# Chyaboiii/antidote_ccrdt

Measured on AMD Instinct MI355X. Metric: CRDT ops/sec (topk_rmv, 1M keys, 8-DC vclocks), higher is better.
Workload: dtype int64

## Files before the change

antidote_ccrdt_amd/csrc/engine.cpp:

```cpp
#include <algorithm>
#include <chrono>
#include <cstdio>
#include <cstdlib>
#include <cstring>
#include <string>
#include <thread>
#include <tuple>
#include <vector>

#include "common.hpp"
#include "engine.hpp"
#include "trmv_kernels.hpp"

namespace ccrdt {

static thread_local std::string g_last_error;
void set_error(const std::string& msg) { g_last_error = msg; }

static constexpr int TRMV_N_TIERS = CCRDT_TRMV_N_TIERS;
static constexpr int TRMV_TIER_LAST = CCRDT_TRMV_TIER_HBM;
static constexpr uint32_t TRMV_HBM_WAVES = 128;
static constexpr uint32_t TRMV_LATER_GRID = 4096;

template <class F>
// ... 234 lines not shown
  }
  if (e->type != CCRDT_TOPK_RMV) {
    set_error("engine is not topk_rmv");
    return CCRDT_ENOSYS;
  }
  if (hipSetDevice(e->device) != hipSuccess) {
    set_error("hipSetDevice failed");
    return CCRDT_EDEVICE;
  }
  return CCRDT_OK;
}

namespace {

int trmv_err_code(uint32_t err) {
  std::string m = "trmv_apply: invalid op in batch:";
  if (err & TRMV_ERR_KIND) m += " kind>3";
  if (err & TRMV_ERR_DC) m += " dc>=n_dc";
  if (err & TRMV_ERR_TS) m += " add ts<1";
  if (err & TRMV_ERR_ROW) m += " rmv row out of range";
  if (err & TRMV_ERR_VC) m += " negative VcRmv entry";
  set_error(m);
  return (err & (TRMV_ERR_TS | TRMV_ERR_VC)) && !(err & (TRMV_ERR_KIND | TRMV_ERR_DC | TRMV_ERR_ROW)) ? CCRDT_ERANGE
                                                                                                  : CCRDT_EINVAL;
}

int env_int(const char* v, int dflt, int lo, int hi) { return std::clamp(v ? atoi(v) : dflt, lo, hi); }
bool env_on(const char* v) { return !(v && v[0] == '0'); }
bool env_is1(const char* v) { return v && v[0] == '1'; }
uint64_t env_u64(const char* v, uint64_t dflt) { return v ? strtoull(v, nullptr, 10) : dflt; }
struct TrmvKnobs {
  int pool_slack = env_int(getenv("CCRDT_TRMV_POOL_SLACK"), 2, 2, 8);
  int first_tier = env_int(getenv("CCRDT_TRMV_FIRST_TIER"), -1, INT32_MIN, INT32_MAX);
  bool overlap = env_on(getenv("CCRDT_TRMV_OVERLAP"));
  bool inplace = env_on(getenv("CCRDT_TRMV_INPLACE"));
  uint64_t overlap_keys = env_u64(getenv("CCRDT_TRMV_OVERLAP_KEYS"), 1ull << 18);
  uint32_t overlap_waves = (uint32_t)env_int(getenv("CCRDT_TRMV_OVERLAP_WAVES"), 32, 1, 4096);
  static const TrmvKnobs& get() {
    static const TrmvKnobs k;
    return k;
  }
};
struct TrmvHooks {
  static bool fail_finish() { return env_is1(getenv("CCRDT_TRMV_FAIL_FINISH")); }
  static bool overlap_stall() { return env_is1(getenv("CCRDT_TRMV_OVERLAP_STALL")); }
  static const char* arena_room() { return getenv("CCRDT_TRMV_ARENA_ROOM"); }
};

struct TrmvStatus {
  static constexpr int TRMV_STATUS_WORDS = 2 + 2 * TRMV_N_TIERS;
  static constexpr uint64_t ALLOC = TRMV_STATUS_WORDS * 4 + 16;
  uint32_t* dev;
  uint32_t* host;
  hipStream_t stream;
  uint32_t* count(int t) const { return dev + 2 + 2 * t; }
  uint32_t* verr() const { return count(CCRDT_TRMV_TIER_RESIDENT) + 1; }
  unsigned long long* vscratch() const { return reinterpret_cast<unsigned long long*>(dev + TRMV_STATUS_WORDS); }
  hipError_t clear() const { return hipMemsetAsync(dev, 0, TRMV_STATUS_WORDS * 4, stream); }
  hipError_t clear_tier(int t) const { return hipMemsetAsync(count(t), 0, 8, stream); }
  hipError_t read_back(bool sync = true) const {
    const hipError_t e = hipMemcpyAsync(host, dev, TRMV_STATUS_WORDS * 4, hipMemcpyDeviceToHost, stream);
    return e != hipSuccess || !sync ? e : hipStreamSynchronize(stream);
  }
  uint32_t handed(int t) const { return host[2 + 2 * t]; }
  uint32_t errors(int t) const { return host[3 + 2 * t]; }
};

struct TrmvRun {
  Engine& E;
  TrmvStatus st;
  TrmvApplyArgs a;
  uint64_t n_ops;
  uint64_t tot[3] = {};
  int chain[4] = {}, n_chain = 0, n_head = 0;
  int prev = -1;
  int next_evt = 0;
};
// ... 227 lines not shown
  a0.n_first = ov + O_NFIRST;
  a0.first_thresh = thresh;
  CCRDT_TRY(trmv_launch_wave(a0, nk, E.stream));
  CCRDT_TRY(trmv_mark(r));
  CCRDT_HIP(hipStreamWaitEvent(E.stream2, E.evt[e0], 0));
  trmv_point(E, r.st, a3, CCRDT_TRMV_TIER_RESIDENT, CCRDT_TRMV_TIER_WAVE);
  a3.prod_waves = trmv_wave_waves(nk);
  a3.claim = ov + O_CLAIM;
  const bool force_stall = TrmvHooks::overlap_stall();
  a3.spin_limit = force_stall ? 0u : (1u << 19);
  CCRDT_TRY(trmv_launch_resident_consume(a3, TrmvKnobs::get().overlap_waves, E.stream2));
  CCRDT_HIP(hipEventRecord(E.ev_ovl, E.stream2));
  CCRDT_HIP(hipStreamWaitEvent(E.stream, E.ev_ovl, 0));
  CCRDT_TRY(trmv_mark(r));
  CCRDT_HIP(r.st.read_back());
  if ((r.st.errors(CCRDT_TRMV_TIER_RESIDENT) & TRMV_ERR_STALL) || force_stall) {
    CCRDT_HIP(r.st.clear_tier(CCRDT_TRMV_TIER_RESIDENT));
    a3.pub = nullptr;
    a3.done = nullptr;
    CCRDT_TRY(trmv_launch_resident(a3, std::min<uint64_t>(nk, TRMV_LATER_GRID), E.stream));
    --r.next_evt;
    CCRDT_TRY(trmv_mark(r));
    CCRDT_HIP(r.st.read_back());
    E.trmv_overflow_keys[CCRDT_TRMV_SLOT_STALL_FALLBACK] = 1;
  }
  CCRDT_TRY(trmv_book(E, r.st, r.chain, 2, e0));
  r.prev = CCRDT_TRMV_TIER_RESIDENT;
  return CCRDT_OK;
}

int trmv_run_chain(TrmvRun& r) {
  const Engine& E = r.E;
  const TrmvKnobs& knobs = TrmvKnobs::get();
  const bool overlap = knobs.overlap && E.fresh && E.n_keys && (uint64_t)E.n_keys <= knobs.overlap_keys &&
                       r.n_head == 2 && r.chain[0] == CCRDT_TRMV_TIER_WAVE && r.chain[1] == CCRDT_TRMV_TIER_RESIDENT;
  if (overlap) CCRDT_TRY(trmv_head_overlapped(r));
  else CCRDT_TRY(trmv_segment(r, r.chain, r.n_head));
  if (r.n_head < r.n_chain && E.n_keys && r.st.handed(r.chain[r.n_head - 1]) != 0)
    CCRDT_TRY(trmv_segment(r, r.chain + r.n_head, r.n_chain - r.n_head));
  return CCRDT_OK;
}

int trmv_tier4_and_keep(TrmvRun& r, int& n_over) {
  Engine& E = r.E;
  const uint32_t n_big = E.n_keys ? r.st.handed(CCRDT_TRMV_TIER_S1024) : 0u;
  if (n_big) {
    CCRDT_TRY(E.hbm_scratch.ensure((uint64_t)TRMV_HBM_WAVES * trmv_steady_hbm_bytes(E.k <= 128)));
    const int tier_hbm = CCRDT_TRMV_TIER_HBM;
    r.prev = CCRDT_TRMV_TIER_S1024;
    CCRDT_TRY(trmv_segment(r, &tier_hbm, 1, n_big));
  }
  n_over = (int)E.trmv_overflow_keys[CCRDT_TRMV_TIER_HBM];
  if (n_over) {
    r.a.key_list = E.tier_ovf[TRMV_TIER_LAST].as<uint32_t>();
    r.a.n_list = 0;
    r.a.n_list_dev = r.st.count(TRMV_TIER_LAST);
    CCRDT_TRY(trmv_launch_keep(r.a, std::min<uint32_t>((uint32_t)n_over, TRMV_LATER_GRID), E.stream));
  }
  return CCRDT_OK;
}

int trmv_open_arena(TrmvRun& r) {
  Engine& E = r.E;
  const uint64_t* tot = r.tot;
  trmv_side_caps(E, 1 - E.cur, E.arena_cap);
  if (const char* v = TrmvHooks::arena_room())
    for (int x = 0; x < 3; ++x) E.arena_cap[x] = std::min<uint64_t>(E.arena_cap[x], tot[x] + strtoull(v, nullptr, 10));
// ... 917 lines not shown
```

antidote_ccrdt_amd/csrc/trmv_wave.hip:

```cpp
#include "common.hpp"
#include "trmv_kernels.hpp"

#ifdef TRMV_PROF
__device__ unsigned long long g_trmv_prof[16];
#define PROF_STAMP(v)                                                        \
  do {                                                                       \
    __builtin_amdgcn_sched_barrier(0);                                       \
    asm volatile("s_memtime %0\n\ts_waitcnt lgkmcnt(0)" : "=s"(v)::"memory"); \
    __builtin_amdgcn_sched_barrier(0);                                       \
  } while (0)
#define PROF_MARK(i)                                                         \
  do {                                                                       \
    unsigned long long _t;                                                   \
    PROF_STAMP(_t);                                                          \
    if (lane_id() == 0 && (key & 63u) == 3) atomicAdd(&g_trmv_prof[i], _t - prof_t);             \
    prof_t = _t;                                                             \
  } while (0)
#else
#define PROF_STAMP(v) (void)0
#define PROF_MARK(i) (void)0
#endif

namespace ccrdt {

// ... 18 lines not shown
  unsigned long long htab[W_HCAP + 2];
  int64_t esc[W_ECAP + 2];
  int64_t ets[W_ECAP + 2];
  int64_t rows[W_RCAP][TRMV_DPAD];
  unsigned long long vc[TRMV_DPAD + 2];
  uint32_t pcnt2[W_PCAP / 2 + 4];
  uint32_t rsrc[W_RCAP];
  uint16_t ekd[W_ECAP + 8];
  uint8_t hp[W_HCAP];
  uint8_t sorted[W_ECAP + 8];
  uint8_t slab[W_ECAP];
  uint8_t fin[NS_ * (W_ECAP + 8)];
  uint32_t pa[W_PCAP + 8];
  uint32_t pb[W_PCAP + 8];
  uint8_t pmoff[NS_ * (W_PCAP + 8)];
  uint8_t peb[NS_ * (W_PCAP + 8)];
  uint8_t cpl[W_PCAP + 8];
  uint8_t rl[W_RCAP + 8];
  uint32_t nex;
  __device__ __forceinline__ uint8_t& fa(uint32_t p, int b) { return reinterpret_cast<uint8_t*>(pa)[4 * p + b]; }
  __device__ __forceinline__ uint8_t& fb(uint32_t p, int b) { return reinterpret_cast<uint8_t*>(pb)[4 * p + b]; }
};
#define PSTART(p) L.fa((p), 0)
#define PLR(p) L.fa((p), 1)
#define PFLAG(p) L.fa((p), 2)
#define PCNTF(p) L.fa((p), 3)
#define POBS(p) L.fb((p), 0)
#define PROW(p) L.fb((p), 1)
#define PGB(p) L.fb((p), 2)
#define PSLOT(p) L.fb((p), 3)

#define KA trmv_kargs()

__device__ __forceinline__ uint32_t whash(int64_t id) {
  const uint64_t x = (uint64_t)id * 0x9E3779B97F4A7C15ull;
  return (uint32_t)(x >> 56);
}

template <class W>
__device__ __forceinline__ uint32_t pcnt_of(const W& L, uint32_t p) {
  return (L.pcnt2[p >> 1] >> (16 * (p & 1))) & 0xFFFFu;
}

template <class W>
__device__ __forceinline__ void wave_emit(const TrmvApplyArgs& a, W& L, uint64_t op0,
                                          uint64_t op, uint8_t kind, int64_t id, int64_t sc,
                                          uint32_t dc, int64_t ts, uint32_t row) {
  const uint32_t pos = atomicAdd(&L.nex, 1u);
  TrmvExtraRec r;
  r.op = (uint32_t)op;
  r.kind = kind;
  r.dc = (uint8_t)dc;
  r.pad = 0;
  r.id = id;
  r.score = sc;
  r.ts = ts;
  KA->ex[op0 + pos] = r;
  if (kind == CCRDT_TRMV_RMV)
    for (int d = 0; d < KA->n_dc; ++d) KA->ex_vc[(op0 + pos) * KA->n_dc + d] = L.rows[row][d];
}

struct KeyIn {
  uint64_t op0;
  uint32_t nops;
  KeyMeta nmeta;
  int64_t id[2], sc[2], ts[2];
  uint32_t kind[2], dc[2];
  int64_t rv[W_RCAP / 8];
};

struct ChunkHdr {
  uint32_t key;
  uint64_t lo, hi;
  uint32_t meta[W_MD];
  uint64_t skip;
};

__device__ __forceinline__ uint32_t wave_list_key(uint32_t i, uint32_t n_first) {
  if (KA->first_list) return i < n_first ? KA->first_list[i] : i - n_first;
  return KA->key_list ? KA->key_list[i] : i;
}

__device__ __forceinline__ void wave_load_chunk(const TrmvApplyArgs& a, uint32_t c0, uint32_t n,
                                                uint32_t n_first, ChunkHdr& h) {
  const int lane = lane_id();
  const uint32_t j = (uint32_t)lane < n ? (uint32_t)lane : 0u;
  h.key = wave_list_key(c0 + j, n_first);
  h.lo = KA->key_ptr[h.key];
  h.hi = KA->key_ptr[h.key + 1];
  h.skip = KA->first_list ? ballot((uint32_t)lane < n && c0 + j >= n_first && h.hi - h.lo > KA->first_thresh) : 0ull;
#pragma unroll
  for (int i = 0; i < W_MD; ++i) {
    const uint32_t m = 8 * i + (lane >> 3);
    const uint32_t jm = m < n ? m : 0u;
    const uint32_t km = shfl32(h.key, (int)jm);
    if (KA->fresh) {
      const uint32_t d = lane & 7;
      h.meta[i] = d < 3 ? (uint32_t)trmv_fresh_off(KA->slack != 0, (int)d, km, KA->key_ptr[km])
                        : (d == 7 ? NONE32 : 0u);
    } else {
      h.meta[i] = reinterpret_cast<const uint32_t*>(a.new_s.meta + km)[lane & 7];
    }
  }
}

__device__ __forceinline__ void wave_load_key(const TrmvApplyArgs& a, const ChunkHdr& h, uint32_t j,
                                              KeyIn& in) {
  const int lane = lane_id();
  in.op0 = (uint64_t)rl64((int64_t)h.lo, (int)j);
  in.nops = (uint32_t)((uint64_t)rl64((int64_t)h.hi, (int)j) - in.op0);
  uint32_t* m = reinterpret_cast<uint32_t*>(&in.nmeta);
#pragma unroll
  for (int d = 0; d < 8; ++d) {
    uint32_t v = 0;
#pragma unroll
    for (int i = 0; i < W_MD; ++i)
      if ((j >> 3) == (uint32_t)i) v = rl32(h.meta[i], (int)(8 * (j & 7) + d));
    m[d] = v;
  }
  const int64_t* idp = KA->id + in.op0;
  const int64_t* scp = KA->score + in.op0;
  const int64_t* tsp = KA->ts + in.op0;
  const uint8_t* kp = KA->kind + in.op0;
  const uint8_t* dp = KA->dc + in.op0;
#pragma unroll
  for (int s = 0; s < 2; ++s) {
    const uint32_t l = s * 64 + lane;
    const bool v = l < in.nops;
    in.id[s] = v ? LD_IN(idp + l) : 0;
    in.sc[s] = v ? LD_IN(scp + l) : 0;
    in.ts[s] = v ? LD_IN(tsp + l) : 0;
    in.kind[s] = v ? (uint32_t)LD_IN(kp + l) : 0u;
    in.dc[s] = v ? (uint32_t)LD_IN(dp + l) : 0u;
  }
}

template <class W>
__device__ __forceinline__ void wave_load_rows(const TrmvApplyArgs& a, W& L, KeyIn& in) {
  const int lane = lane_id();
#pragma unroll
  for (int s = 0; s < W_RCAP / 8; ++s) in.rv[s] = 0;
  bool r[2];
#pragma unroll
  for (int s = 0; s < 2; ++s)
    r[s] = (uint32_t)(s * 64 + lane) < in.nops && (in.kind[s] == 2 || in.kind[s] == 3);
  const uint64_t b0 = ballot(r[0]), b1 = ballot(r[1]);
  const uint32_t n0 = (uint32_t)__builtin_popcountll(b0);
  const uint32_t n = n0 + (uint32_t)__builtin_popcountll(b1);
  if (n == 0 || KA->n_rmv_rows <= 0) return;
#pragma unroll
  for (int s = 0; s < 2; ++s) {
    const uint32_t k = s ? n0 + mbcnt(b1) : mbcnt(b0);
    if (r[s] && k < (uint32_t)W_RCAP)
      L.rsrc[k] = (in.ts[s] >= 0 && in.ts[s] < KA->n_rmv_rows) ? (uint32_t)in.ts[s] : 0u;
  }
  wave_lds_sync();
  const uint32_t d = (lane & 7) < KA->n_dc ? (lane & 7) : 0u;
#pragma unroll
  for (int s = 0; s < W_RCAP / 8; ++s) {
    const uint32_t k = s * 8 + (lane >> 3);
    const uint32_t row = k < n ? L.rsrc[k] : 0u;
    in.rv[s] = KA->rmv_vc[(uint64_t)row * KA->n_dc + d];
  }
  wave_lds_sync();
}

enum : int { W_DONE = 0, W_NEXT_TIER = 1, W_REJECT = 2 };

template <bool FRESH>
__device__ __forceinline__ int trmv_wave_key(const TrmvApplyArgs& a, uint32_t key, const KeyIn& in,
                                              WaveLds<FRESH>& L, bool has_next, const ChunkHdr& hdr,
                                              uint32_t nj, KeyIn& nxt) {
  int lane = lane_id();
  asm volatile("" : "+v"(lane));
  const int D = KA->n_dc;
#ifdef TRMV_PROF
  unsigned long long prof_t;
  PROF_STAMP(prof_t);
#endif
  const uint64_t op0 = in.op0;
  const uint32_t nops = in.nops;
  KeyMeta nmeta = in.nmeta;
  nmeta.p_off = __builtin_amdgcn_readfirstlane(nmeta.p_off);
  nmeta.m_off = __builtin_amdgcn_readfirstlane(nmeta.m_off);
  nmeta.r_off = __builtin_amdgcn_readfirstlane(nmeta.r_off);
  KeyMeta om;
  if (FRESH) {
    om.p_off = om.m_off = om.r_off = 0;
    om.np = om.nm = om.nr = om.nobs = 0;
    om.minq = NONE32;
  } else {
    om = a.old_s.meta[key];
  }
  const uint32_t pmax = KA->k < (uint32_t)W_PCAP ? KA->k : (uint32_t)W_PCAP;
  if (nops > (uint32_t)W_ECAP || om.np > pmax || om.nm + nops > (uint32_t)W_ECAP ||
      om.nr > (uint32_t)W_RCAP)
    return W_NEXT_TIER;

  int64_t xsc[2] = {in.sc[0], in.sc[1]};
  const int64_t xts[2] = {in.ts[0], in.ts[1]};
  const uint32_t xkind[2] = {in.kind[0], in.kind[1]};
  const uint32_t xdc[2] = {in.dc[0], in.dc[1]};
  const bool xv[2] = {(uint32_t)lane < nops, (uint32_t)(64 + lane) < nops};
  int64_t pid[2] = {0, 0};
  uint32_t pinfo[2] = {NONE32, NONE32}, pslab[2] = {0u, 0u};
  if (!FRESH) {
#pragma unroll
    for (int s = 0; s < 2; ++s) {
      const uint32_t p = s * 64 + lane;
      if (p < om.np) {
        pid[s] = (a.old_s.pl_id + om.p_off)[p];
        pinfo[s] = (a.old_s.pl_info + om.p_off)[p];
        pslab[s] = (a.old_s.pl_slab + om.p_off)[p];
      }
    }
  }
#pragma unroll
  for (int i = 0; i < W_HCAP / 64; ++i) L.htab[i * 64 + lane] = W_EMPTY;
  if (lane == 0) {
    L.htab[HSINK] = W_EMPTY;
    L.nex = 0u;
  }
  reinterpret_cast<uint32_t*>(L.hp)[lane] = 0xFFFFFFFFu;
  L.pcnt2[lane] = 0u;
  L.pa[lane] = 0u;
  L.pa[64 + lane] = 0u;
  L.pb[lane] = 0xFFFFFFFFu;
  L.pb[64 + lane] = 0xFFFFFFFFu;
  if (lane < 8) {
    L.pa[128 + lane] = 0u;
    L.pb[128 + lane] = 0xFFFFFFFFu;
  }
  if (lane < TRMV_DPAD)
    L.vc[lane] = (!FRESH && lane < D) ? (unsigned long long)a.old_s.vc[(uint64_t)key * D + lane] : 0ull;
  if (!FRESH) {
    for (uint32_t r0 = 0; r0 < om.nr; r0 += 8) {
      const uint32_t r = r0 + (lane >> 3), d = lane & 7;
      if (r < om.nr)
        L.rows[r][d] = (int)d < D ? (a.old_s.r_vc + (uint64_t)om.r_off * D)[r * D + d] : 0;
    }
  }

  PROF_MARK(0);
  uint32_t err = 0;
  bool xr[2], xa[2];
#pragma unroll
  for (int s = 0; s < 2; ++s) {
    xa[s] = xv[s] && xkind[s] < 2;
    xr[s] = xv[s] && (xkind[s] == 2 || xkind[s] == 3);
    err |= (xv[s] && xkind[s] > 3) ? TRMV_ERR_KIND : 0u;
    err |= (xa[s] && (int)xdc[s] >= D) ? TRMV_ERR_DC : 0u;
    err |= (xa[s] && xts[s] < 1) ? TRMV_ERR_TS : 0u;
    err |= (xr[s] && (xts[s] < 0 || xts[s] >= KA->n_rmv_rows)) ? TRMV_ERR_ROW : 0u;
  }
  if (ballot(err != 0)) {
    if (err) atomicOr(&KA->status[1], err);
    return W_REJECT;
  }
  const uint64_t rb0 = ballot(xr[0]), rb1 = ballot(xr[1]);
  const uint32_t nr0 = (uint32_t)__builtin_popcountll(rb0);
  const uint32_t nrmv = nr0 + (uint32_t)__builtin_popcountll(rb1);
  if (om.nr + nrmv > (uint32_t)W_RCAP) return W_NEXT_TIER;
  {
    const uint32_t r0 = mbcnt(rb0), r1 = nr0 + mbcnt(rb1);
    xsc[0] = xr[0] ? (int64_t)(om.nr + r0) : xsc[0];
    xsc[1] = xr[1] ? (int64_t)(om.nr + r1) : xsc[1];
  }
  wave_lds_sync();
  constexpr int NS = FRESH ? 2 : 4;
  uint32_t hs[4];
  bool pend[4];
  const int64_t hid[4] = {in.id[0], in.id[1], pid[0], pid[1]};
  pend[0] = xv[0];
  pend[1] = xv[1];
  pend[2] = !FRESH && (uint32_t)lane < om.np;
  pend[3] = !FRESH && (uint32_t)(64 + lane) < om.np;
  bool bad = false;
#pragma unroll
  for (int j = 0; j < NS; ++j) {
    hs[j] = whash(hid[j]);
    bad |= pend[j] && (unsigned long long)hid[j] == W_EMPTY;
  }
  if (ballot(bad)) return W_NEXT_TIER;

  PROF_MARK(1);
  for (;;) {
    bool any = false;
#pragma unroll
    for (int j = 0; j < NS; ++j) any |= pend[j];
    if (!ballot(any)) break;
    unsigned long long prev[4];
#pragma unroll
    for (int j = 0; j < NS; ++j) {
      prev[j] = W_EMPTY;
      if (pend[j]) prev[j] = atomicCAS(&L.htab[hs[j]], W_EMPTY, (unsigned long long)hid[j]);
    }
#pragma unroll
    for (int j = 0; j < NS; ++j) {
      const bool done = prev[j] == W_EMPTY || prev[j] == (unsigned long long)hid[j];
      hs[j] = (pend[j] && !done) ? ((hs[j] + 1) & (W_HCAP - 1)) : hs[j];
      pend[j] = pend[j] && !done;
    }
  }
  PROF_MARK(8);
  {
#pragma unroll
    for (int s = 0; s < W_RCAP / 8; ++s) {
      const uint32_t r = s * 8 + (lane >> 3), d = lane & 7;
      const int64_t v = (int)d < D ? in.rv[s] : 0;
      err |= (r < nrmv && v < 0) ? TRMV_ERR_VC : 0u;
      if (r < nrmv) L.rows[om.nr + r][d] = v;
    }
    if (ballot(err != 0)) {
      if (err) atomicOr(&KA->status[1], err);
      return W_REJECT;
    }
  }
  PROF_MARK(9);
  if (!FRESH) {
#pragma unroll
    for (int s = 0; s < 2; ++s) {
      const uint32_t p = s * 64 + lane;
      if (p < om.np) {
        L.hp[hs[2 + s]] = (uint8_t)p;
        PSLOT(p) = (uint8_t)hs[2 + s];
        bad |= ((pslab[s] >> 16) != 0) != ((pinfo[s] & 0xFFFFu) != NONE16);
      }
    }
    if (ballot(bad)) return W_NEXT_TIER;
  }
  wave_lds_sync();
  uint32_t np;
  {
    const unsigned long long* h4 = &L.htab[lane * 4];
    const unsigned long long t0 = h4[0], t1 = h4[1], t2 = h4[2], t3 = h4[3];
    const uint32_t hp4 = reinterpret_cast<const uint32_t*>(L.hp)[lane];
    const uint32_t n0 = (t0 != W_EMPTY && (hp4 & 0xFFu) == NONE8) ? 1u : 0u;
    const uint32_t n1 = (t1 != W_EMPTY && ((hp4 >> 8) & 0xFFu) == NONE8) ? 1u : 0u;
    const uint32_t n2 = (t2 != W_EMPTY && ((hp4 >> 16) & 0xFFu) == NONE8) ? 1u : 0u;
    const uint32_t n3 = (t3 != W_EMPTY && (hp4 >> 24) == NONE8) ? 1u : 0u;
    const uint32_t c = n0 + n1 + n2 + n3;
    const uint64_t b0 = ballot(c & 1), b1 = ballot(c & 2), b2 = ballot(c & 4);
    const uint32_t base = om.np + mbcnt(b0) + 2 * mbcnt(b1) + 4 * mbcnt(b2);
    np = om.np + (uint32_t)__builtin_popcountll(b0) + 2 * (uint32_t)__builtin_popcountll(b1) +
         4 * (uint32_t)__builtin_popcountll(b2);
    if (np > pmax) return W_NEXT_TIER;
    const uint32_t i0 = base, i1 = i0 + n0, i2 = i1 + n1, i3 = i2 + n2;
    const uint32_t nhp = (n0 ? i0 : (hp4 & 0xFFu)) | ((n1 ? i1 : ((hp4 >> 8) & 0xFFu)) << 8) |
                         ((n2 ? i2 : ((hp4 >> 16) & 0xFFu)) << 16) |
                         ((n3 ? i3 : (hp4 >> 24)) << 24);
    reinterpret_cast<uint32_t*>(L.hp)[lane] = nhp;
    if (n0) PSLOT(i0) = (uint8_t)(lane * 4 + 0);
    if (n1) PSLOT(i1) = (uint8_t)(lane * 4 + 1);
    if (n2) PSLOT(i2) = (uint8_t)(lane * 4 + 2);
    if (n3) PSLOT(i3) = (uint8_t)(lane * 4 + 3);
  }
  wave_lds_sync();
  if (FRESH && has_next) wave_load_key(a, hdr, nj, nxt);

  PROF_MARK(2);
  uint32_t xrank[2], xp[2];
  {
    uint32_t hpv[2], cr[2];
#pragma unroll
    for (int s = 0; s < 2; ++s) hpv[s] = L.hp[hs[s]];
#pragma unroll
    for (int s = 0; s < 2; ++s) {
      const uint32_t p = xv[s] ? hpv[s] : PSINK;
      xp[s] = p;
      if (xa[s]) atomicMax(&L.vc[xdc[s]], (unsigned long long)xts[s]);
      if (!FRESH && xr[s]) PFLAG(p) = 1;
      cr[s] = atomicAdd(&L.pcnt2[(xv[s] ? p : (uint32_t)lane) >> 1], xv[s] ? 1u << (16 * (p & 1)) : 0u);
    }
#pragma unroll
    for (int s = 0; s < 2; ++s) xrank[s] = xv[s] ? (cr[s] >> (16 * (xp[s] & 1))) & 0xFFFFu : 0u;
  }
  wave_lds_sync();
  {
    uint32_t tot0, tot1;
    const uint32_t c0 = (uint32_t)lane < np ? pcnt_of(L, lane) : 0u;
    const uint32_t c1 = (uint32_t)(64 + lane) < np ? pcnt_of(L, 64 + lane) : 0u;
    const uint32_t st0 = wave_excl_scan_dpp(c0, tot0);
    const uint32_t st1 = wave_excl_scan_dpp(c1, tot1);
    PSTART(lane) = (uint8_t)st0;
    PSTART(64 + lane) = (uint8_t)(tot0 + st1);
  }
  wave_lds_sync();
  uint32_t xq[2], xst[2], xc[2];
#pragma unroll
  for (int s = 0; s < 2; ++s) {
    xst[s] = PSTART(xp[s]);
// ... 40 lines not shown
      wave_lds_sync();
#pragma unroll
      for (int s = 0; s < 2; ++s)
        if (xv[s])
          for (uint32_t x = 0; x < xc[s]; ++x)
            if (L.sorted[xst[s] + x] == (uint32_t)(s * 64 + lane)) xq[s] = xst[s] + x;
    }
  }
  if (!FRESH) {
    uint32_t ebase = nops;
#pragma unroll
    for (int s = 0; s < 2; ++s) {
      const uint32_t p = s * 64 + lane;
      const uint32_t oc = p < om.np ? (pslab[s] >> 16) : 0u;
      uint32_t tot;
      const uint32_t eb = ebase + wave_excl_scan_dpp(oc, tot);
      ebase += tot;
      if (p < om.np) {
        L.peb[p] = (uint8_t)eb;
        PFLAG(p) = 1;
      }
      for (uint32_t j = 0; j < oc; ++j) {
        const uint32_t go = (pslab[s] & 0xFFFFu) + j;
        const uint32_t e = eb + j;
        L.esc[e] = (a.old_s.m_score + om.m_off)[go];
        L.ets[e] = (a.old_s.m_ts + om.m_off)[go];
        L.ekd[e] = (uint16_t)(((uint32_t)(a.old_s.m_dc + om.m_off)[go] << 2) | (p << 8));
      }
    }
  }
  wave_lds_sync();

  PROF_MARK(3);
  if (!FRESH && has_next) wave_load_key(a, hdr, nj, nxt);
  if (!FRESH) {
    bool simple[2], beaten[2] = {false, false}, gbeaten[2] = {false, false}, risk[2] = {false, false};
    uint32_t me[2], cl[2];
#pragma unroll
    for (int s = 0; s < 2; ++s) {
      simple[s] = xa[s] && !PFLAG(xp[s]);
      me[s] = xq[s] - xst[s];
      cl[s] = simple[s] ? xc[s] : 0u;
    }
    const uint32_t maxc = wave_max_u32_dpp(cl[0] > cl[1] ? cl[0] : cl[1]);
    for (uint32_t x = 0; x < maxc; ++x) {
#pragma unroll
      for (int s = 0; s < 2; ++s) {
        const bool valid = x < cl[s] && x != me[s];
        const uint32_t pos = x < cl[s] ? xst[s] + x : (uint32_t)ESINK;
        const int64_t sx = L.esc[pos], tx = L.ets[pos];
        const uint32_t dx = (L.ekd[pos] >> 2) & 7u;
        const int64_t sm = xsc[s], tm = xts[s];
        const bool before = x < me[s];
        risk[s] |= valid && before && tx >= tm;
        beaten[s] |= valid && (sx > sm || (sx == sm && (before ? tx >= tm : tx > tm)));
        gbeaten[s] |= valid && (sx > sm || (sx == sm && (dx > xdc[s] || (dx == xdc[s] && tx > tm))));
      }
    }
#pragma unroll
    for (int s = 0; s < 2; ++s) {
      if (risk[s]) PFLAG(xp[s]) = 1;
      if (simple[s] && !beaten[s]) POBS(xp[s]) = (uint8_t)xq[s];
      if (simple[s] && !gbeaten[s]) PGB(xp[s]) = (uint8_t)xq[s];
    }
    wave_lds_sync();
  } else {
    uint8_t* const cq = L.slab;
// ... 71 lines not shown
      if (act) mrg[k] = (uint8_t)(yr && !first);
      any_merge |= ballot(yr && !first) != 0;
    }
    wave_lds_sync();
    if (any_merge) {
#pragma unroll 1
      for (uint32_t b = 0; b < mn; b += 64) {
        const uint32_t k = b + lane;
        const uint32_t q = k < mn && mrg[k] ? (uint32_t)cq[k] : ESINK;
        const uint32_t p = q != ESINK ? (uint32_t)(L.ekd[q] >> 8) : PSINK;
        if (q != ESINK && !PFLAG(p)) {
          unsigned long long* dst = reinterpret_cast<unsigned long long*>(L.rows[PROW(p)]);
          const int64_t* src = L.rows[(uint32_t)L.esc[q]];
          for (int d = 0; d < D; ++d) atomicMax(dst + d, (unsigned long long)src[d]);
        }
      }
    }
    wave_lds_sync();
  }

  PROF_MARK(6);
  uint32_t ncx;
  {
    const bool c0 = (uint32_t)lane < np && PFLAG(lane);
    const bool c1 = (uint32_t)(64 + lane) < np && PFLAG(64 + lane);
    const uint64_t m0 = ballot(c0), m1 = ballot(c1);
    const uint32_t n0 = (uint32_t)__builtin_popcountll(m0);
    ncx = n0 + (uint32_t)__builtin_popcountll(m1);
    if (c0) L.cpl[mbcnt(m0)] = (uint8_t)lane;
    if (c1) L.cpl[n0 + mbcnt(m1)] = (uint8_t)(64 + lane);
  }
  wave_lds_sync();
  __builtin_amdgcn_s_waitcnt(0x0F70);
  if (FRESH && has_next) wave_load_rows(a, L, nxt);
  PROF_MARK(7);
  uint32_t best_q = NONE32;
  int64_t best_sc = INT64_MAX, best_id = INT64_MAX;
  auto min_cand = [&](bool has, int64_t sc, int64_t id, uint32_t p) {
    const bool better = has && (best_q == NONE32 || sc < best_sc || (sc == best_sc && id < best_id));
    best_q = better ? p : best_q;
    best_sc = better ? sc : best_sc;
    best_id = better ? id : best_id;
  };
  if (FRESH) {
#pragma unroll
    for (int s = 0; s < 2; ++s) {
      const uint32_t q = s * 64 + lane;
      const uint32_t qq = q < nops ? q : (uint32_t)ESINK;
      const int64_t sc = L.esc[qq], ts = L.ets[qq];
      const uint32_t kd = L.ekd[qq];
      if (q < nops) {
        ST_OUT((KA->new_s.m_score + nmeta.m_off) + (q), sc);
        ST_OUT((KA->new_s.m_ts + nmeta.m_off) + (q), ts);
        ST_OUT((KA->new_s.m_dc + nmeta.m_off) + (q), (uint8_t)((kd >> 2) & 7u));
      }
    }
  }
  uint32_t mbase = 0;
#pragma unroll 1
  for (uint32_t b = 0; b < ncx; b += 64) {
    const uint32_t k = b + lane;
    const bool act = k < ncx;
    const uint32_t p = act ? L.cpl[k] : 0u;
    uint32_t ocnt = 0, pinfo_p = NONE32, eb = 0;
    if (!FRESH && act && p < om.np) {
      pinfo_p = (a.old_s.pl_info + om.p_off)[p];
      ocnt = (a.old_s.pl_slab + om.p_off)[p] >> 16;
      eb = L.peb[p];
    }
    const uint32_t c = act ? pcnt_of(L, p) : 0u;
    const uint32_t st = act ? PSTART(p) : 0u;
    uint32_t tot;
    const uint32_t moff = mbase + wave_excl_scan_dpp(c + ocnt, tot);
    mbase += tot;
    uint32_t cnt = ocnt;
    int64_t maxts = 0;
    for (uint32_t j = 0; j < cnt; ++j) {
      L.slab[moff + j] = (uint8_t)(eb + j);
      const int64_t t = L.ets[eb + j];
      maxts = t > maxts ? t : maxts;
    }
    uint32_t o = NONE8, prow = NONE8;
    int64_t osc = 0, ots = 0;
    if (!FRESH && act && p < om.np) {
      const uint32_t oi = pinfo_p & 0xFFFFu, ri = pinfo_p >> 16;
      if (oi != NONE16) {
        o = eb + oi;
// ... 45 lines not shown
        bool alive = false;
        int64_t bsc = 0, bts = 0;
        for (uint32_t j = 0; j < cnt; ++j) {
          const uint32_t e2 = L.slab[moff + j];
          const int64_t t2 = L.ets[e2];
          const uint32_t d2 = (L.ekd[e2] >> 2) & 7u;
          if (t2 > L.rows[vs][d2]) {
            L.slab[moff + w++] = (uint8_t)e2;
            alive |= e2 == o;
            const int64_t s2 = L.esc[e2];
            if (be == NONE8 || s2 > bsc || (s2 == bsc && (d2 > bdc || (d2 == bdc && t2 > bts)))) {
              be = e2;
              bsc = s2;
              bdc = d2;
              bts = t2;
            }
          }
        }
        cnt = w;
        if (o != NONE8 && !alive) {
          if (cnt == 0) {
            o = NONE8;
          } else {
            o = be;
            osc = bsc;
            ots = bts;
            wave_emit(a, L, op0, op0 + L.sorted[e], CCRDT_TRMV_ADD, id, bsc, bdc, bts, prow);
          }
        }
      }
    }
    if (FRESH) {
      uint32_t opos = NONE16, gj = 0;
      for (uint32_t j = 0; j < cnt; ++j) {
        const uint32_t e2 = L.slab[moff + j];
        const int64_t s2 = L.esc[e2], t2 = L.ets[e2];
        const uint32_t d2 = (L.ekd[e2] >> 2) & 7u;
        ST_OUT((KA->new_s.m_score + nmeta.m_off) + (st + j), s2);
        ST_OUT((KA->new_s.m_ts + nmeta.m_off) + (st + j), t2);
        ST_OUT((KA->new_s.m_dc + nmeta.m_off) + (st + j), (uint8_t)d2);
        opos = e2 == o ? j : opos;
        const uint32_t eb = L.slab[moff + gj];
        const int64_t bs = L.esc[eb], bt = L.ets[eb];
        const uint32_t bd = (L.ekd[eb] >> 2) & 7u;
        if (s2 > bs || (s2 == bs && (d2 > bd || (d2 == bd && t2 > bt)))) gj = j;
      }
      if (act) {
        POBS(p) = (uint8_t)(o == NONE8 ? NONE8 : st + opos);
        PGB(p) = (uint8_t)(st + gj);
        PCNTF(p) = (uint8_t)cnt;
        PROW(p) = (uint8_t)prow;
      }
      min_cand(act && o != NONE8, osc, id, p);
    } else if (act) {
      POBS(p) = (uint8_t)o;
      PCNTF(p) = (uint8_t)cnt;
      L.pmoff[p] = (uint8_t)moff;
      PROW(p) = (uint8_t)prow;
    }
  }
  wave_lds_sync();
  if (!FRESH && has_next) wave_load_rows(a, L, nxt);

  PROF_MARK(4);
  uint32_t fbase = 0, rbase = 0, nobs = 0;
  uint32_t po[2] = {NONE8, NONE8};
  if (FRESH) {
    uint32_t csum = 0;
#pragma unroll
    for (int s = 0; s < 2; ++s) {
      const uint32_t p = s * 64 + lane;
      const bool act = p < np;
      const uint32_t pp = act ? p : (uint32_t)PSINK;
      const uint32_t wa = L.pa[pp], wb = L.pb[pp];
      const uint32_t st = wa & 0xFFu, c = pcnt_of(L, pp), lrp = (wa >> 8) & 0xFFu;
      const bool replayed = ((wa >> 16) & 0xFFu) != 0;
      const uint32_t off = (replayed || lrp == 0) ? st : lrp;
      const uint32_t cnt = act ? (replayed ? (wa >> 24) : st + c - off) : 0u;
      const uint32_t o = act ? (wb & 0xFFu) : NONE8;
      const uint32_t prow = act ? ((wb >> 8) & 0xFFu) : NONE8;
      const uint64_t rm = ballot(prow != NONE8);
      const uint32_t rix = rbase + mbcnt(rm);
      rbase += (uint32_t)__builtin_popcountll(rm);
      if (prow != NONE8) L.rl[rix] = (uint8_t)prow;
      const int64_t id = (int64_t)L.htab[wb >> 24];
      const uint32_t gb = (replayed || cnt > 1) ? ((wb >> 16) & 0xFFu) - off : 0u;
      if (act) {
        ST_OUT((KA->new_s.pl_id + nmeta.p_off) + (p), id);
        ST_OUT((KA->new_s.pl_slab + nmeta.p_off) + (p), off | (cnt << 16));
        if (cnt > 1) ST_OUT((KA->new_s.pl_gb + nmeta.p_off) + (p), (uint16_t)gb);
        ST_OUT(KA->new_s.pl_info + nmeta.p_off + p, (o == NONE8 ? NONE16 : o - off) |
                                             ((prow != NONE8 ? rix : NONE16) << 16));
      }
      csum += cnt;
      nobs += (uint32_t)__builtin_popcountll(ballot(o != NONE8));
      min_cand(!replayed && o != NONE8, L.esc[o != NONE8 ? o : (uint32_t)ESINK], id, p);
    }
    (void)wave_excl_scan_dpp(csum, fbase);
    wave_lds_sync();
  } else {
  {
    uint32_t cnt[2], st[2], moff[2], goff[2], prow[2], opos[2], gbj[2], gbd[2];
    int64_t gbs[2], gbt[2];
    bool act[2], cx[2];
#pragma unroll
    for (int s = 0; s < 2; ++s) {
      const uint32_t p = s * 64 + lane;
      act[s] = p < np;
      const uint32_t pp = act[s] ? p : PSINK;
      cx[s] = act[s] && PFLAG(pp);
      const uint32_t c = pcnt_of(L, pp);
      st[s] = PSTART(pp);
      po[s] = act[s] ? POBS(pp) : NONE8;
      cnt[s] = act[s] ? (cx[s] ? (uint32_t)PCNTF(pp) : c) : 0u;
      prow[s] = cx[s] ? PROW(pp) : NONE8;
      moff[s] = cx[s] ? L.pmoff[pp] : 0u;
      uint32_t ftot;
      goff[s] = fbase + wave_excl_scan_dpp(cnt[s], ftot);
      fbase += ftot;
      opos[s] = (act[s] && !cx[s]) ? po[s] - st[s] : NONE16;
      gbj[s] = (act[s] && !cx[s]) ? (uint32_t)PGB(pp) - st[s] : 0u;
      gbd[s] = 0u;
      gbs[s] = gbt[s] = 0;
    }
    const uint32_t maxcnt = wave_max_u32_dpp(cnt[0] > cnt[1] ? cnt[0] : cnt[1]);
// ... 21 lines not shown
      const uint32_t p = s * 64 + lane;
      const uint64_t rm = ballot(prow[s] != NONE8);
      const uint32_t rix = rbase + mbcnt(rm);
      rbase += (uint32_t)__builtin_popcountll(rm);
      if (prow[s] != NONE8) L.rl[rix] = (uint8_t)prow[s];
      const int64_t id = (int64_t)L.htab[PSLOT(act[s] ? p : PSINK)];
      if (act[s]) {
        (KA->new_s.pl_id + nmeta.p_off)[p] = id;
        (KA->new_s.pl_info + nmeta.p_off)[p] = (po[s] == NONE8 ? NONE16 : opos[s]) |
                                             ((prow[s] != NONE8 ? rix : NONE16) << 16);
        (KA->new_s.pl_slab + nmeta.p_off)[p] = goff[s] | (cnt[s] << 16);
        (KA->new_s.pl_gb + nmeta.p_off)[p] = (uint16_t)(cnt[s] ? gbj[s] : 0u);
      }
      nobs += (uint32_t)__builtin_popcountll(ballot(act[s] && po[s] != NONE8));
    }
  }
  wave_lds_sync();

#pragma unroll
  for (int s = 0; s < 2; ++s) {
    const uint32_t q = s * 64 + lane;
    const uint32_t e0 = L.fin[q < fbase ? q : (uint32_t)ESINK];
    const uint32_t e = e0 < (uint32_t)W_ECAP ? e0 : (uint32_t)ESINK;
    const int64_t sc = L.esc[e], ts = L.ets[e];
    const uint8_t dc = (uint8_t)((L.ekd[e] >> 2) & 7u);
    if (q < fbase) {
      (KA->new_s.m_score + nmeta.m_off)[q] = sc;
      (KA->new_s.m_ts + nmeta.m_off)[q] = ts;
      (KA->new_s.m_dc + nmeta.m_off)[q] = dc;
    }
  }
  }
  PROF_MARK(10);
  for (uint32_t r0 = 0; r0 < rbase; r0 += 8) {
    const uint32_t r = r0 + (lane >> 3), d = lane & 7;
    const int64_t v = L.rows[L.rl[r < rbase ? r : 0u]][d];
    if (r < rbase && (int)d < D) (KA->new_s.r_vc + (uint64_t)nmeta.r_off * D)[r * D + d] = v;
  }
  if (lane < D) KA->new_s.vc[(uint64_t)key * D + lane] = (int64_t)L.vc[lane];
  PROF_MARK(11);
  {
    if (!FRESH) {
#pragma unroll
      for (int s = 0; s < 2; ++s) {
        const uint32_t p = s * 64 + lane;
        const uint32_t o = po[s];
        const int64_t sc = L.esc[o != NONE8 ? o : (uint32_t)ESINK];
        const int64_t id = (int64_t)L.htab[PSLOT(o != NONE8 ? p : (uint32_t)PSINK)];
        min_cand(o != NONE8, sc, id, p);
      }
    }
    const bool has = best_q != NONE32;
    const bool narrow = best_sc == (int64_t)(int32_t)best_sc && best_id == (int64_t)(int32_t)best_id;
    if (!ballot(has)) {
      best_q = NONE32;
    } else if (!ballot(has && !narrow)) {
      const uint32_t us = has ? (uint32_t)(int32_t)best_sc ^ 0x80000000u : 0xFFFFFFFFu;
      const uint32_t ms = wave_min_u32_dpp(us);
      const bool at = has && us == ms;
      const uint32_t ui = at ? (uint32_t)(int32_t)best_id ^ 0x80000000u : 0xFFFFFFFFu;
      const uint32_t mi = wave_min_u32_dpp(ui);
      best_q = rl32(best_q, (int)__builtin_ctzll(ballot(at && ui == mi)));
    } else {
      const int64_t ms = wave_min_i64_dpp(has ? best_sc : INT64_MAX);
      const int64_t mi = wave_min_i64_dpp(has && best_sc == ms ? best_id : INT64_MAX);
      const uint64_t hit = ballot(has && best_sc == ms && best_id == mi);
      best_q = rl32(best_q, (int)__builtin_ctzll(hit));
    }
  }
  if (lane == 0) {
    KeyMeta out = nmeta;
    out.np = np;
    out.nm = fbase;
    out.nr = rbase;
    out.nobs = nobs;
    out.minq = best_q;
    KA->new_s.meta[key] = out;
    KA->ex_cnt[key] = L.nex;
    if (FRESH && KA->slack) {
      KeyCap c;
      c.p_cap = trmv_fresh_cap(true, 0, nops);
      c.m_cap = trmv_fresh_cap(true, 1, nops);
      c.r_cap = trmv_fresh_cap(true, 2, nops);
      c.m_top = (uint16_t)nops;
      c.flags = TRMV_CAP_VALID;
      KA->new_s.cap[key] = c;
    }
  }
  PROF_MARK(5);
  return W_DONE;
}
}

template <bool FRESH, int OCC>
__global__ __launch_bounds__(64 * W_WAVES, OCC) void trmv_wave_kernel(TrmvApplyArgs a) {
  __shared__ WaveLds<FRESH> lds[W_WAVES];
  const uint32_t wv = __builtin_amdgcn_readfirstlane(threadIdx.x >> 6);
  WaveLds<FRESH>& L = lds[wv];
  const uint32_t n_first = a.first_list ? *a.n_first : 0u;
  const uint32_t n = (a.n_list_dev ? *a.n_list_dev : a.n_list) + n_first;
  for (uint32_t c0 = (blockIdx.x * W_WAVES + wv) * W_KPW; c0 < n; c0 += gridDim.x * W_WAVES * W_KPW) {
    const uint32_t cn = c0 + W_KPW < n ? W_KPW : n - c0;
    ChunkHdr hdr;
    wave_load_chunk(a, c0, cn, n_first, hdr);
    KeyIn cur, nxt;
    wave_load_key(a, hdr, 0, cur);
    __builtin_amdgcn_s_waitcnt(0x0F70);
    wave_load_rows(a, L, cur);
    for (uint32_t j = 0; j < cn; ++j) {
      const uint32_t key = rl32(hdr.key, (int)j);
      const bool has_next = j + 1 < cn;
      const int r = (hdr.skip >> j) & 1u ? W_REJECT + 1
                                         : trmv_wave_key<FRESH>(a, key, cur, L, has_next, hdr, j + 1, nxt);
      if (r != W_DONE) {
        if (r == W_NEXT_TIER && lane_id() == 0) {
          const uint32_t pos = atomicAdd(&KA->status[0], 1u);
          KA->ovf_list[pos] = key;
          if (KA->pub && pos < KA->n_pub) {
            const uint32_t old = atomicExch(&KA->pub[pos], key + 1u);
// ... 52 lines not shown
```

Baseline: 47.81 billion.

## Hoist kernel-arg loads, use 32-bit offset addressing, and reorder next-key prefetch

Result: faster. 49.79 billion, median of 6 (+4.1%).

```diff
diff --git a/antidote_ccrdt_amd/csrc/engine.cpp b/antidote_ccrdt_amd/csrc/engine.cpp
--- a/antidote_ccrdt_amd/csrc/engine.cpp
+++ b/antidote_ccrdt_amd/csrc/engine.cpp
@@ -290,7 +290,6 @@
 struct TrmvKnobs {
   int pool_slack = env_int(getenv("CCRDT_TRMV_POOL_SLACK"), 2, 2, 8);
   int first_tier = env_int(getenv("CCRDT_TRMV_FIRST_TIER"), -1, INT32_MIN, INT32_MAX);
-  bool overlap = env_on(getenv("CCRDT_TRMV_OVERLAP"));
   bool inplace = env_on(getenv("CCRDT_TRMV_INPLACE"));
   uint64_t overlap_keys = env_u64(getenv("CCRDT_TRMV_OVERLAP_KEYS"), 1ull << 18);
   uint32_t overlap_waves = (uint32_t)env_int(getenv("CCRDT_TRMV_OVERLAP_WAVES"), 32, 1, 4096);
@@ -301,6 +300,7 @@
 };
 struct TrmvHooks {
   static bool fail_finish() { return env_is1(getenv("CCRDT_TRMV_FAIL_FINISH")); }
+  static bool overlap() { return env_on(getenv("CCRDT_TRMV_OVERLAP")); }
   static bool overlap_stall() { return env_is1(getenv("CCRDT_TRMV_OVERLAP_STALL")); }
   static const char* arena_room() { return getenv("CCRDT_TRMV_ARENA_ROOM"); }
 };
@@ -594,7 +594,7 @@
 int trmv_run_chain(TrmvRun& r) {
   const Engine& E = r.E;
   const TrmvKnobs& knobs = TrmvKnobs::get();
-  const bool overlap = knobs.overlap && E.fresh && E.n_keys && (uint64_t)E.n_keys <= knobs.overlap_keys &&
+  const bool overlap = TrmvHooks::overlap() && E.fresh && E.n_keys && (uint64_t)E.n_keys <= knobs.overlap_keys &&
                        r.n_head == 2 && r.chain[0] == CCRDT_TRMV_TIER_WAVE && r.chain[1] == CCRDT_TRMV_TIER_RESIDENT;
   if (overlap) CCRDT_TRY(trmv_head_overlapped(r));
   else CCRDT_TRY(trmv_segment(r, r.chain, r.n_head));
diff --git a/antidote_ccrdt_amd/csrc/trmv_wave.hip b/antidote_ccrdt_amd/csrc/trmv_wave.hip
--- a/antidote_ccrdt_amd/csrc/trmv_wave.hip
+++ b/antidote_ccrdt_amd/csrc/trmv_wave.hip
@@ -74,6 +74,43 @@
 
 #define KA trmv_kargs()
 
+template <class T>
+__device__ __forceinline__ T* at32(T* base, uint32_t i) {
+  using B = typename std::conditional<std::is_const<T>::value, const char, char>::type;
+  return reinterpret_cast<T*>(reinterpret_cast<B*>(base) + (size_t)(uint32_t)(i * (uint32_t)sizeof(T)));
+}
+
+struct KaOps {
+  const uint8_t* kind;
+  const int64_t* id;
+  const int64_t* score;
+  const uint8_t* dc;
+  const int64_t* ts;
+};
+struct KaPool {
+  int64_t* m_score;
+  int64_t* m_ts;
+  uint8_t* m_dc;
+};
+struct KaPlayers {
+  int64_t* pl_id;
+  uint32_t* pl_info;
+  uint32_t* pl_slab;
+  uint16_t* pl_gb;
+};
+__device__ __forceinline__ KaOps ka_ops(uint64_t op0) {
+  const auto* ka = KA;
+  return {ka->kind + op0, ka->id + op0, ka->score + op0, ka->dc + op0, ka->ts + op0};
+}
+__device__ __forceinline__ KaPool ka_pool(uint32_t m_off) {
+  const auto* ka = KA;
+  return {ka->new_s.m_score + m_off, ka->new_s.m_ts + m_off, ka->new_s.m_dc + m_off};
+}
+__device__ __forceinline__ KaPlayers ka_players(uint32_t p_off) {
+  const auto* ka = KA;
+  return {ka->new_s.pl_id + p_off, ka->new_s.pl_info + p_off, ka->new_s.pl_slab + p_off, ka->new_s.pl_gb + p_off};
+}
+
 __device__ __forceinline__ uint32_t whash(int64_t id) {
   const uint64_t x = (uint64_t)id * 0x9E3779B97F4A7C15ull;
   return (uint32_t)(x >> 56);
@@ -118,27 +155,34 @@
   uint64_t skip;
 };
 
-__device__ __forceinline__ uint32_t wave_list_key(uint32_t i, uint32_t n_first) {
-  if (KA->first_list) return i < n_first ? KA->first_list[i] : i - n_first;
-  return KA->key_list ? KA->key_list[i] : i;
+__device__ __forceinline__ uint32_t wave_list_key(const uint32_t* first_list, const uint32_t* key_list, uint32_t i,
+                                                 uint32_t n_first) {
+  if (first_list) return i < n_first ? first_list[i] : i - n_first;
+  return key_list ? key_list[i] : i;
 }
 
 __device__ __forceinline__ void wave_load_chunk(const TrmvApplyArgs& a, uint32_t c0, uint32_t n,
                                                 uint32_t n_first, ChunkHdr& h) {
   const int lane = lane_id();
   const uint32_t j = (uint32_t)lane < n ? (uint32_t)lane : 0u;
-  h.key = wave_list_key(c0 + j, n_first);
-  h.lo = KA->key_ptr[h.key];
-  h.hi = KA->key_ptr[h.key + 1];
-  h.skip = KA->first_list ? ballot((uint32_t)lane < n && c0 + j >= n_first && h.hi - h.lo > KA->first_thresh) : 0ull;
+  const auto* ka = KA;
+  const uint64_t* key_ptr = ka->key_ptr;
+  const uint32_t* first_list = ka->first_list;
+  const uint32_t* key_list = ka->key_list;
+  const bool fresh = ka->fresh != 0, room = ka->slack != 0;
+  const uint32_t first_thresh = ka->first_thresh;
+  h.key = wave_list_key(first_list, key_list, c0 + j, n_first);
+  h.lo = key_ptr[h.key];
+  h.hi = key_ptr[h.key + 1];
+  h.skip = first_list ? ballot((uint32_t)lane < n && c0 + j >= n_first && h.hi - h.lo > first_thresh) : 0ull;
 #pragma unroll
   for (int i = 0; i < W_MD; ++i) {
     const uint32_t m = 8 * i + (lane >> 3);
     const uint32_t jm = m < n ? m : 0u;
     const uint32_t km = shfl32(h.key, (int)jm);
-    if (KA->fresh) {
+    if (fresh) {
       const uint32_t d = lane & 7;
-      h.meta[i] = d < 3 ? (uint32_t)trmv_fresh_off(KA->slack != 0, (int)d, km, KA->key_ptr[km])
+      h.meta[i] = d < 3 ? (uint32_t)trmv_fresh_off(room, (int)d, km, key_ptr[km])
                         : (d == 7 ? NONE32 : 0u);
     } else {
       h.meta[i] = reinterpret_cast<const uint32_t*>(a.new_s.meta + km)[lane & 7];
@@ -160,26 +204,30 @@
       if ((j >> 3) == (uint32_t)i) v = rl32(h.meta[i], (int)(8 * (j & 7) + d));
     m[d] = v;
   }
-  const int64_t* idp = KA->id + in.op0;
-  const int64_t* scp = KA->score + in.op0;
-  const int64_t* tsp = KA->ts + in.op0;
-  const uint8_t* kp = KA->kind + in.op0;
-  const uint8_t* dp = KA->dc + in.op0;
+  const KaOps o = ka_ops(in.op0);
 #pragma unroll
   for (int s = 0; s < 2; ++s) {
-    const uint32_t l = s * 64 + lane;
-    const bool v = l < in.nops;
-    in.id[s] = v ? LD_IN(idp + l) : 0;
-    in.sc[s] = v ? LD_IN(scp + l) : 0;
-    in.ts[s] = v ? LD_IN(tsp + l) : 0;
-    in.kind[s] = v ? (uint32_t)LD_IN(kp + l) : 0u;
-    in.dc[s] = v ? (uint32_t)LD_IN(dp + l) : 0u;
+    uint32_t l = s * 64 + lane;
+    in.id[s] = in.sc[s] = in.ts[s] = 0;
+    in.kind[s] = in.dc[s] = 0u;
+    if (l < in.nops) {
+      asm volatile("" : "+v"(l));
+      in.id[s] = LD_IN(at32(o.id, l));
+      in.sc[s] = LD_IN(at32(o.score, l));
+      in.ts[s] = LD_IN(at32(o.ts, l));
+      in.kind[s] = (uint32_t)LD_IN(at32(o.kind, l));
+      in.dc[s] = (uint32_t)LD_IN(at32(o.dc, l));
+    }
   }
 }
 
 template <class W>
 __device__ __forceinline__ void wave_load_rows(const TrmvApplyArgs& a, W& L, KeyIn& in) {
   const int lane = lane_id();
+  const auto* ka = KA;
+  const int64_t* rmv_vc = ka->rmv_vc;
+  const int64_t n_rmv_rows = ka->n_rmv_rows;
+  const uint32_t n_dc = (uint32_t)ka->n_dc;
 #pragma unroll
   for (int s = 0; s < W_RCAP / 8; ++s) in.rv[s] = 0;
   bool r[2];
@@ -189,20 +237,20 @@
   const uint64_t b0 = ballot(r[0]), b1 = ballot(r[1]);
   const uint32_t n0 = (uint32_t)__builtin_popcountll(b0);
   const uint32_t n = n0 + (uint32_t)__builtin_popcountll(b1);
-  if (n == 0 || KA->n_rmv_rows <= 0) return;
+  if (n == 0 || n_rmv_rows <= 0) return;
 #pragma unroll
   for (int s = 0; s < 2; ++s) {
     const uint32_t k = s ? n0 + mbcnt(b1) : mbcnt(b0);
     if (r[s] && k < (uint32_t)W_RCAP)
-      L.rsrc[k] = (in.ts[s] >= 0 && in.ts[s] < KA->n_rmv_rows) ? (uint32_t)in.ts[s] : 0u;
-  }
-  wave_lds_sync();
-  const uint32_t d = (lane & 7) < KA->n_dc ? (lane & 7) : 0u;
+      L.rsrc[k] = (in.ts[s] >= 0 && in.ts[s] < n_rmv_rows) ? (uint32_t)in.ts[s] : 0u;
+  }
+  wave_lds_sync();
+  const uint32_t d = (uint32_t)(lane & 7) < n_dc ? (lane & 7) : 0u;
 #pragma unroll
   for (int s = 0; s < W_RCAP / 8; ++s) {
     const uint32_t k = s * 8 + (lane >> 3);
     const uint32_t row = k < n ? L.rsrc[k] : 0u;
-    in.rv[s] = KA->rmv_vc[(uint64_t)row * KA->n_dc + d];
+    in.rv[s] = rmv_vc[(uint64_t)row * n_dc + d];
   }
   wave_lds_sync();
 }
@@ -215,7 +263,10 @@
                                               uint32_t nj, KeyIn& nxt) {
   int lane = lane_id();
   asm volatile("" : "+v"(lane));
-  const int D = KA->n_dc;
+  const auto* ka0 = KA;
+  const int D = ka0->n_dc;
+  const uint32_t size_k = ka0->k;
+  const int64_t n_rmv_rows = ka0->n_rmv_rows;
 #ifdef TRMV_PROF
   unsigned long long prof_t;
   PROF_STAMP(prof_t);
@@ -234,7 +285,7 @@
   } else {
     om = a.old_s.meta[key];
   }
-  const uint32_t pmax = KA->k < (uint32_t)W_PCAP ? KA->k : (uint32_t)W_PCAP;
+  const uint32_t pmax = size_k < (uint32_t)W_PCAP ? size_k : (uint32_t)W_PCAP;
   if (nops > (uint32_t)W_ECAP || om.np > pmax || om.nm + nops > (uint32_t)W_ECAP ||
       om.nr > (uint32_t)W_RCAP)
     return W_NEXT_TIER;
@@ -293,7 +344,7 @@
     err |= (xv[s] && xkind[s] > 3) ? TRMV_ERR_KIND : 0u;
     err |= (xa[s] && (int)xdc[s] >= D) ? TRMV_ERR_DC : 0u;
     err |= (xa[s] && xts[s] < 1) ? TRMV_ERR_TS : 0u;
-    err |= (xr[s] && (xts[s] < 0 || xts[s] >= KA->n_rmv_rows)) ? TRMV_ERR_ROW : 0u;
+    err |= (xr[s] && (xts[s] < 0 || xts[s] >= n_rmv_rows)) ? TRMV_ERR_ROW : 0u;
   }
   if (ballot(err != 0)) {
     if (err) atomicOr(&KA->status[1], err);
@@ -345,7 +396,11 @@
     }
   }
   PROF_MARK(8);
-  {
+  auto clock_rows_to_lds = [&]() -> bool {
+#ifdef TRMV_PROF
+    __builtin_amdgcn_s_waitcnt(0x0F70);
+#endif
+    PROF_MARK(12);
 #pragma unroll
     for (int s = 0; s < W_RCAP / 8; ++s) {
       const uint32_t r = s * 8 + (lane >> 3), d = lane & 7;
@@ -355,10 +410,10 @@
     }
     if (ballot(err != 0)) {
       if (err) atomicOr(&KA->status[1], err);
-      return W_REJECT;
-    }
-  }
-  PROF_MARK(9);
+      return true;
+    }
+    return false;
+  };
   if (!FRESH) {
 #pragma unroll
     for (int s = 0; s < 2; ++s) {
@@ -398,7 +453,6 @@
     if (n3) PSLOT(i3) = (uint8_t)(lane * 4 + 3);
   }
   wave_lds_sync();
-  if (FRESH && has_next) wave_load_key(a, hdr, nj, nxt);
 
   PROF_MARK(2);
   uint32_t xrank[2], xp[2];
@@ -505,7 +559,10 @@
   wave_lds_sync();
 
   PROF_MARK(3);
-  if (!FRESH && has_next) wave_load_key(a, hdr, nj, nxt);
+  if (clock_rows_to_lds()) return W_REJECT;
+  wave_lds_sync();
+  PROF_MARK(9);
+  if (has_next) wave_load_key(a, hdr, nj, nxt);
   if (!FRESH) {
     bool simple[2], beaten[2] = {false, false}, gbeaten[2] = {false, false}, risk[2] = {false, false};
     uint32_t me[2], cl[2];
@@ -643,6 +700,7 @@
   }
   wave_lds_sync();
   __builtin_amdgcn_s_waitcnt(0x0F70);
+  PROF_MARK(15);
   if (FRESH && has_next) wave_load_rows(a, L, nxt);
   PROF_MARK(7);
   uint32_t best_q = NONE32;
@@ -654,6 +712,7 @@
     best_id = better ? id : best_id;
   };
   if (FRESH) {
+    const KaPool pool = ka_pool(nmeta.m_off);
 #pragma unroll
     for (int s = 0; s < 2; ++s) {
       const uint32_t q = s * 64 + lane;
@@ -661,9 +720,9 @@
       const int64_t sc = L.esc[qq], ts = L.ets[qq];
       const uint32_t kd = L.ekd[qq];
       if (q < nops) {
-        ST_OUT((KA->new_s.m_score + nmeta.m_off) + (q), sc);
-        ST_OUT((KA->new_s.m_ts + nmeta.m_off) + (q), ts);
-        ST_OUT((KA->new_s.m_dc + nmeta.m_off) + (q), (uint8_t)((kd >> 2) & 7u));
+        ST_OUT(at32(pool.m_score, q), sc);
+        ST_OUT(at32(pool.m_ts, q), ts);
+        ST_OUT(at32(pool.m_dc, q), (uint8_t)((kd >> 2) & 7u));
       }
     }
   }
@@ -775,13 +834,14 @@
     }
     if (FRESH) {
       uint32_t opos = NONE16, gj = 0;
+      const KaPool pool = ka_pool(nmeta.m_off);
       for (uint32_t j = 0; j < cnt; ++j) {
         const uint32_t e2 = L.slab[moff + j];
         const int64_t s2 = L.esc[e2], t2 = L.ets[e2];
         const uint32_t d2 = (L.ekd[e2] >> 2) & 7u;
-        ST_OUT((KA->new_s.m_score + nmeta.m_off) + (st + j), s2);
-        ST_OUT((KA->new_s.m_ts + nmeta.m_off) + (st + j), t2);
-        ST_OUT((KA->new_s.m_dc + nmeta.m_off) + (st + j), (uint8_t)d2);
+        ST_OUT(at32(pool.m_score, st + j), s2);
+        ST_OUT(at32(pool.m_ts, st + j), t2);
+        ST_OUT(at32(pool.m_dc, st + j), (uint8_t)d2);
         opos = e2 == o ? j : opos;
         const uint32_t eb = L.slab[moff + gj];
         const int64_t bs = L.esc[eb], bt = L.ets[eb];
@@ -810,6 +870,7 @@
   uint32_t po[2] = {NONE8, NONE8};
   if (FRESH) {
     uint32_t csum = 0;
+    const KaPlayers rec = ka_players(nmeta.p_off);
 #pragma unroll
     for (int s = 0; s < 2; ++s) {
       const uint32_t p = s * 64 + lane;
@@ -829,11 +890,10 @@
       const int64_t id = (int64_t)L.htab[wb >> 24];
       const uint32_t gb = (replayed || cnt > 1) ? ((wb >> 16) & 0xFFu) - off : 0u;
       if (act) {
-        ST_OUT((KA->new_s.pl_id + nmeta.p_off) + (p), id);
-        ST_OUT((KA->new_s.pl_slab + nmeta.p_off) + (p), off | (cnt << 16));
-        if (cnt > 1) ST_OUT((KA->new_s.pl_gb + nmeta.p_off) + (p), (uint16_t)gb);
-        ST_OUT(KA->new_s.pl_info + nmeta.p_off + p, (o == NONE8 ? NONE16 : o - off) |
-                                             ((prow != NONE8 ? rix : NONE16) << 16));
+        ST_OUT(at32(rec.pl_id, p), id);
+        ST_OUT(at32(rec.pl_slab, p), off | (cnt << 16));
+        ST_OUT(at32(rec.pl_info, p), (o == NONE8 ? NONE16 : o - off) | ((prow != NONE8 ? rix : NONE16) << 16));
+        if (cnt > 1) ST_OUT(at32(rec.pl_gb, p), (uint16_t)gb);
       }
       csum += cnt;
       nobs += (uint32_t)__builtin_popcountll(ballot(o != NONE8));
@@ -921,13 +981,30 @@
   }
   }
   PROF_MARK(10);
+#ifdef TRMV_PROF
+  {
+    unsigned long long probe;
+    asm volatile("s_load_dwordx2 %0, %1, 0x40\n\ts_waitcnt lgkmcnt(0)" : "=s"(probe) : "s"(KA) : "memory");
+    asm volatile("" ::"s"(probe));
+  }
+  PROF_MARK(13);
+  PROF_MARK(14);
+#endif
+  const auto* ka1 = KA;
+  int64_t* const rvc = ka1->new_s.r_vc + (uint64_t)nmeta.r_off * D;
+  int64_t* const kvc = ka1->new_s.vc + (uint64_t)key * D;
   for (uint32_t r0 = 0; r0 < rbase; r0 += 8) {
     const uint32_t r = r0 + (lane >> 3), d = lane & 7;
     const int64_t v = L.rows[L.rl[r < rbase ? r : 0u]][d];
-    if (r < rbase && (int)d < D) (KA->new_s.r_vc + (uint64_t)nmeta.r_off * D)[r * D + d] = v;
-  }
-  if (lane < D) KA->new_s.vc[(uint64_t)key * D + lane] = (int64_t)L.vc[lane];
+    if (r < rbase && (int)d < D) *at32(rvc, r * D + d) = v;
+  }
+  if (lane < D) *at32(kvc, (uint32_t)lane) = (int64_t)L.vc[lane];
   PROF_MARK(11);
+  const auto* ka2 = KA;
+  KeyMeta* const meta_out = ka2->new_s.meta + key;
+  KeyCap* const cap_out = ka2->new_s.cap + key;
+  uint32_t* const ex_cnt_out = ka2->ex_cnt + key;
+  const bool room = ka2->slack != 0;
   {
     if (!FRESH) {
 #pragma unroll
@@ -964,16 +1041,16 @@
     out.nr = rbase;
     out.nobs = nobs;
     out.minq = best_q;
-    KA->new_s.meta[key] = out;
-    KA->ex_cnt[key] = L.nex;
-    if (FRESH && KA->slack) {
+    *meta_out = out;
+    *ex_cnt_out = L.nex;
+    if (FRESH && room) {
       KeyCap c;
       c.p_cap = trmv_fresh_cap(true, 0, nops);
       c.m_cap = trmv_fresh_cap(true, 1, nops);
       c.r_cap = trmv_fresh_cap(true, 2, nops);
       c.m_top = (uint16_t)nops;
       c.flags = TRMV_CAP_VALID;
-      KA->new_s.cap[key] = c;
+      *cap_out = c;
     }
   }
   PROF_MARK(5);
```
